# NoahVl/Explaining-In-Style-Reproducibility-Study

Hardware: AMD Instinct MI355X
Metric: StylEx G+D+enc train-step images/sec @256px (higher is better)
Workload: dtype bf16; 1 GPU; FFHQ-shaped 256x256 StylEx, batch 32/GPU, GAE=2 (noise+encoder micro-steps), GP every 4th step, ResNet-18 classifier; image_size=256, batch_per_gpu=32, start_step=0, gradient_accumulate_every=2, global_batch=32, parallelism=dp1

## Files before the change

### explaining-in-style-reproducibility-study_amd/csrc/fused_bwd.hip

```cpp
#include <hip/hip_runtime.h>
#include <stdint.h>
#include <stdlib.h>

#include "stylex_internal.h"

namespace {

constexpr int NT = 256;

template <int K>
struct Acc {
    float4 v[K];
    __device__ __forceinline__ void zero() {
#pragma unroll
        for (int k = 0; k < K; ++k) v[k] = make_float4(0.f, 0.f, 0.f, 0.f);
    }
};

template <int K>
__device__ __forceinline__ void block_reduce_store(Acc<K>& a, float* smem, int cv, int prow, int CV, int rpp, int C,
                                                   float* partial_row , bool active) {
    float4* s4 = reinterpret_cast<float4*>(smem);
    if (active) {
#pragma unroll
// ... 441 lines not shown
                        int nchunks, int act_dtype, void* stream) {
    if (act_dtype != 0 && act_dtype != 1) return STYLEX_EINVAL;
    if (!x || !t || !s || !partial || !ok_shape(sh, nchunks)) return STYLEX_EINVAL;
    int HW = (int)(sh[1] * sh[2]), C = (int)sh[3];
    if (glue_wide(act_dtype, C) && al16(x) && al16(t) && al16(s) && al16(gx) && al16(partial)) {
        hipLaunchKernelGGL(scale_reduce_wide_kernel, dim3(nchunks, (unsigned)sh[0]), dim3(NT8), reduce_smem8(C, 1),
                           (hipStream_t)stream, x, t, s, gx, partial, HW, C, nchunks);
        return (int)hipGetLastError();
    }
    hipLaunchKernelGGL(scale_reduce_kernel, dim3(nchunks, (unsigned)sh[0]), dim3(NT), reduce_smem(C, 1),
                       (hipStream_t)stream, x, t, s, gx, partial, HW, C, nchunks, act_dtype);
    return (int)hipGetLastError();
}

}
```

### explaining-in-style-reproducibility-study_amd/stylex/hip_backend.py

```python
import os as _os

if _os.environ.get("STYLEX_MIOPEN_ALLOW_BWD_GTC", "0") != "1":
    _os.environ.setdefault("MIOPEN_DEBUG_CONV_IMPLICIT_GEMM_ASM_BWD_GTC_XDLOPS_NHWC", "0")

import atexit
import ctypes
import os
import weakref

import torch

import operand_cache
from operand_cache import mark_updated, packs, stamp as _gen, vectors

_HERE = os.path.dirname(os.path.abspath(__file__))
LIB_PATH = os.path.join(os.path.dirname(_HERE), "libstylex_hip.so")

F32, BF16, BF16_ACT = 0, 1, 2
EPI_BIAS, EPI_LRELU, EPI_OSCALE, EPI_NOISE, EPI_RESIDUAL, EPI_RELU, EPI_GATE, EPI_NOISE_NAT = 1, 2, 4, 8, 16, 32, 64, 128
EPI_MASK_OUT, EPI_GATE_MASK = 256, 512

_c_f = ctypes.c_void_p
_i64p = ctypes.POINTER(ctypes.c_int64)

# ... 55 lines not shown
    "stylex_bias_act_fwd": (ctypes.c_int, [_c_f, _c_f, _c_f, ctypes.c_int64, _c_f, _c_f, _c_f, _i64p, ctypes.c_int,
                                           ctypes.c_void_p]),
    "stylex_bias_act_bwd": (ctypes.c_int, [_c_f, _c_f, _c_f, _i64p, ctypes.c_int, ctypes.c_void_p]),
    "stylex_rowwise_sumsq": (ctypes.c_int, [_c_f, _c_f, _i64p, ctypes.c_void_p]),
    "stylex_reduce_chunks": (ctypes.c_int, [_i64p]),
    "stylex_act_bwd_reduce": (ctypes.c_int, [_c_f, _c_f, _c_f, _c_f, _i64p, ctypes.c_int, ctypes.c_int, ctypes.c_float,
                                             ctypes.c_int, ctypes.c_void_p]),
    "stylex_modconv_bwd_prep": (ctypes.c_int, [_c_f, _c_f, _c_f, ctypes.c_int64, _c_f, _c_f, _c_f, _c_f, _i64p,
                                               ctypes.c_int, ctypes.c_int, ctypes.c_int, ctypes.c_void_p]),
    "stylex_modconv_bwd_prep_scaled": (ctypes.c_int, [_c_f, _c_f, _c_f, ctypes.c_int64, _c_f, _c_f, _c_f, _c_f, _c_f, _i64p,
                                                      ctypes.c_int, ctypes.c_int, ctypes.c_int, ctypes.c_void_p]),
    "stylex_modconv_bwd_prep_nat": (ctypes.c_int, [_c_f, _c_f, _c_f, ctypes.c_int64, _c_f, _c_f, _c_f, _c_f, _c_f, _i64p,
                                                   ctypes.c_int, ctypes.c_int, ctypes.c_int, ctypes.c_void_p]),
    "stylex_scale_reduce": (ctypes.c_int, [_c_f, _c_f, _c_f, _c_f, _c_f, _i64p, ctypes.c_int, ctypes.c_int,
                                           ctypes.c_void_p]),
    "stylex_pad_rgb8": (ctypes.c_int, [_c_f, _c_f, _i64p, _i64p, ctypes.c_int, ctypes.c_void_p]),
    "stylex_affine_act_nchw_fwd": (ctypes.c_int, [_c_f, _c_f, _c_f, _c_f, _c_f, ctypes.c_int64, ctypes.c_int64, ctypes.c_int64,
                                                  ctypes.c_int, ctypes.c_void_p]),
    "stylex_affine_act_nchw_bwd": (ctypes.c_int, [_c_f, _c_f, _c_f, _c_f, _c_f, ctypes.c_int64, ctypes.c_int64, ctypes.c_int64,
                                                  ctypes.c_int, ctypes.c_void_p]),
    "stylex_affine_relu_maxpool_fwd": (ctypes.c_int, [_c_f, _c_f, _c_f, _c_f, _c_f, ctypes.c_int64, ctypes.c_int64,
                                                      ctypes.c_int64, ctypes.c_int64, ctypes.c_void_p]),
    "stylex_affine_relu_maxpool_bwd": (ctypes.c_int, [_c_f, _c_f, _c_f, _c_f, ctypes.c_int64, ctypes.c_int64, ctypes.c_int64,
                                                      ctypes.c_int64, ctypes.c_void_p]),
    "stylex_lpips_tap_nhwc_fwd": (ctypes.c_int, [_c_f, _c_f, _c_f, _c_f, _c_f, _c_f, ctypes.c_int64, ctypes.c_int64, ctypes.c_int64,
                                                 ctypes.c_int64, ctypes.c_void_p]),
    "stylex_lpips_tap_nhwc_bwd": (ctypes.c_int, [_c_f, _c_f, _c_f, _c_f, _c_f, _c_f, _c_f, _c_f, ctypes.c_int64, ctypes.c_int64,
                                                 ctypes.c_int64, ctypes.c_void_p]),
    "stylex_nchw_f32_to_nhwc_bf16": (ctypes.c_int, [_c_f, _c_f, ctypes.c_int64, ctypes.c_int64, ctypes.c_int64, ctypes.c_int,
                                                    ctypes.c_void_p]),
# ... 86 lines not shown
                                          ctypes.c_int64, _c_f, _c_f, ctypes.c_int64, ctypes.c_void_p]),
    "stylex_style_edit_max_k": (ctypes.c_int64, []),
    "stylex_style_edit_levels": (ctypes.c_int, [_c_f] * 9 + [ctypes.c_int64] * 5 + [ctypes.c_float, ctypes.c_void_p]),
    "stylex_timing_report": (ctypes.c_int, [ctypes.c_int, _i64p, ctypes.POINTER(ctypes.c_double),
                                            ctypes.POINTER(ctypes.c_double), ctypes.POINTER(ctypes.c_double)]),
}

_lib = None
_inited_devices = set()


class StylexHipError(RuntimeError):
    pass


OPTIONAL_SYMBOLS = frozenset(["stylex_modconv_bwd_prep_nat"])
_MISSING_OPTIONAL = set()


def has_symbol(name):
    load_library()
    return name not in _MISSING_OPTIONAL


def load_library(path=None):
    global _lib
    if _lib is not None:
        return _lib
    path = path or os.environ.get("STYLEX_HIP_LIB", LIB_PATH)
    if not os.path.isfile(path):
        raise StylexHipError("libstylex_hip.so not found at %s — run `python __graft_entry__.py build` "
# ... 1448 lines not shown

def torgb_bwd(x, gy, s1, w, want_gx=True):
    lib = _ensure_device(x)
    assert is_cl(x) and is_cl(gy) and gy.shape[1] == 4 and x.dtype == gy.dtype == torch.bfloat16
    b, c, h, wd = x.shape
    shp = _shape(b, h, wd, c)
    nch = lib.stylex_torgb_chunks(shp)
    partial = _empty((b, nch, 3, c), dtype=torch.float32, device=x.device)
    gx = empty_cl(tuple(x.shape), x) if want_gx else None
    s1, w = _f32(s1), _f32(w)
    _check(lib.stylex_torgb_bwd(_ptr(x), _ptr(gy), _ptr(s1), _ptr(w), _ptr(gx), _ptr(partial), shp, _stream()),
           "stylex_torgb_bwd")
    return gx, (partial.sum(dim=1) if nch > 1 else partial[:, 0])


_STYLE_EDIT_MAX_K = None


def style_edit_max_k():
    global _STYLE_EDIT_MAX_K
    if _STYLE_EDIT_MAX_K is None:
        _STYLE_EDIT_MAX_K = int(load_library().stylex_style_edit_max_k())
    return _STYLE_EDIT_MAX_K


def _host_i32(values, what):
    v = [int(i) for i in values]
    if not v:
        raise ValueError("style_edit_levels: %s is empty" % what)
    return v
# ... 293 lines not shown
```

### explaining-in-style-reproducibility-study_amd/stylex/networks.py

```python
import atexit
import math
from math import log2

import os

import torch
import torch.nn.functional as F
from torch import nn

import ops


def exists(v):
    return v is not None


_SIDE = {}
atexit.register(_SIDE.clear)


def _side_stream(t, which=0):
    import os

    if not t.is_cuda or os.environ.get("STYLEX_STREAMS", "1") == "0":
# ... 188 lines not shown
        self.to_style = nn.Linear(latent_dim, input_channel)
        self.conv = Conv2DMod(input_channel, 4 if rgba else 3, 1, demod=False)
        self.upsample = nn.Sequential(Upsample2x(), Blur()) if upsample else None

    def forward(self, x, prev_rgb, istyle, style=None, padded=False):
        style = self.to_style(istyle) if style is None else style
        if padded and not self.conv.demod:
            fused = ops.rgb_block(x, prev_rgb, style, self.conv.weight, exists(self.upsample))
            if fused is not None:
                return fused
        if exists(prev_rgb) and prev_rgb.shape[1] == 4 and self.conv.weight.shape[0] == 3:
            prev_rgb = prev_rgb[:, :3]
        x = self.conv(x, style)
        if exists(prev_rgb):
            x = x + prev_rgb
        if exists(self.upsample):
            x = self.upsample(x)
        return x


class GeneratorBlock(nn.Module):
    def __init__(self, latent_dim, input_channels, filters, upsample=True, upsample_rgb=True, rgba=False):
        super().__init__()
        self.input_channels, self.filters = input_channels, filters
        self.num_style_coords = input_channels + filters
        self.upsample = Upsample2x() if upsample else None
        self.to_style1 = nn.Linear(latent_dim, input_channels)
        self.to_noise1 = nn.Linear(1, filters)
        self.conv1 = Conv2DMod(input_channels, filters, 3)
        self.to_style2 = nn.Linear(latent_dim, filters)
# ... 9 lines not shown
        self._rgb_style = None
        if styles is None:
            fused = ops.style_affines(istyle, self.to_style1, self.to_style2, self.to_rgb.to_style)
            if fused is not None:
                style1, style2, self._rgb_style, coords = fused
            else:
                style1, style2 = self.to_style1(istyle), self.to_style2(istyle)
        else:
            style1, style2 = styles
        x = ops.modconv_noise_act(x, style1, self.conv1.weight, inoise, self.to_noise1.weight[:, 0],
                                  self.to_noise1.bias, demod=self.conv1.demod, eps=self.conv1.eps)
        x = ops.modconv_noise_act(x, style2, self.conv2.weight, inoise, self.to_noise2.weight[:, 0],
                                  self.to_noise2.bias, demod=self.conv2.demod, eps=self.conv2.eps)
        return x, (coords if coords is not None else torch.cat([style1, style2], dim=-1))

    def forward(self, x, prev_rgb, istyle, inoise):
        x, coords = self.forward_main(x, istyle, inoise)
        rgb = self.to_rgb(x, prev_rgb, istyle, style=self.__dict__.pop("_rgb_style", None))
        return x, rgb, coords


class DiscriminatorBlock(nn.Module):
    def __init__(self, input_channels, filters, downsample=True):
        super().__init__()
        self.conv_res = HipConv2d(input_channels, filters, 1, stride=(2 if downsample else 1))
        self.net = nn.Sequential(HipConv2d(input_channels, filters, 3, padding=1, act=True), _FusedAct(),
                                 HipConv2d(filters, filters, 3, padding=1, act=True), _FusedAct())
        self.downsample = nn.Sequential(Blur(), HipConv2d(filters, filters, 3, padding=1, stride=2)) if downsample else None

    def forward(self, x):
        fused = getattr(ops.impl(), "dblock", None)
# ... 53 lines not shown

    def first_activation(self, styles):
        if self.no_const:
            return ops.initial_block(styles, self.to_initial_block.weight)
        return self.initial_block.expand(styles.shape[0], -1, -1, -1)

    def forward(self, styles, input_noise, get_style_coords=False, block_inputs=None):
        x = self.initial_conv(self.first_activation(styles))
        rgb, coords = None, []
        per_layer = styles.unbind(1)
        for li, block in enumerate(self.blocks):
            if exists(self.attns[li]):
                x = self.attns[li](x)
            if block_inputs is not None:
                block_inputs.append((x, rgb))
            x, sc = block.forward_main(x, per_layer[li], input_noise)
            coords.append(sc)
            rgb = block.to_rgb(x, rgb, per_layer[li], style=block.__dict__.pop("_rgb_style", None), padded=True)
        if rgb.shape[1] == 4 and self.blocks[0].to_rgb.conv.filters == 3:
            rgb = rgb[:, :3]
        rgb = rgb.float()
        if get_style_coords:
            return rgb, torch.cat(coords, dim=1)
        return rgb


class DiscriminatorE(nn.Module):
    def __init__(self, image_size, network_capacity=16, fq_layers=[], fq_dict_size=256, attn_layers=[],
                 transparent=False, encoder=False, encoder_dim=512, fmap_max=512, conditional=False):
        super().__init__()
# ... 31 lines not shown
```

### explaining-in-style-reproducibility-study_amd/stylex/ops.py

```python
import collections
import math

import os

import torch
from contextlib import nullcontext as _nullcontext
import torch.nn.functional as F

import hip_backend as hb

_PRECISION = hb.F32


_NAMES = {"fp32": hb.F32, "f32": hb.F32, "bf16": hb.BF16_ACT, "bf16_f32act": hb.BF16}


def set_precision(name):
    global _PRECISION
    _PRECISION = _NAMES[name]


def get_precision():
    return {hb.F32: "fp32", hb.BF16_ACT: "bf16", hb.BF16: "bf16_f32act"}[_PRECISION]

# ... 574 lines not shown


class _RGBTailFast(torch.autograd.Function):

    @staticmethod
    def forward(ctx, rgb, prev):
        return hb.rgb_up_blur_add_fwd(_cl(rgb), _cl(prev) if prev is not None else None)

    @staticmethod
    @torch.autograd.function.once_differentiable
    def backward(ctx, gy):
        g = hb.rgb_up_blur_add_bwd(_cl(gy))
        return g, (g if ctx.needs_input_grad[1] else None)


class _BlurS2D(torch.autograd.Function):

    @staticmethod
    def forward(ctx, x):
        return hb.blur3x3_s2d_fwd(_cl(x))

    @staticmethod
    def backward(ctx, gy2):
        return _BlurS2DBwd.apply(gy2)


class _BlurS2DBwd(torch.autograd.Function):
    @staticmethod
    def forward(ctx, gy2):
        return hb.blur3x3_s2d_bwd(_cl(gy2))
# ... 389 lines not shown
    @staticmethod
    def rgb_block(x, prev_rgb, style, weight, upsample):
        if not fast_enabled() or os.environ.get("STYLEX_RGB_TAIL", "1") == "0":
            return None
        x = _act(x)
        if tuple(weight.shape[2:]) != (1, 1) or weight.shape[0] != 3 or not hb.torgb_ok(x):
            return None
        if prev_rgb is not None and (prev_rgb.shape[1] != 4 or prev_rgb.dtype != x.dtype):
            return None
        rgb = _ToRGBFast.apply(x, style + 1, weight)
        if upsample:
            return _RGBTailFast.apply(rgb, prev_rgb)
        return rgb if prev_rgb is None else rgb + prev_rgb

    @staticmethod
    def residual_merge(x, res):
        return (x + res) * (1 / math.sqrt(2))

    @staticmethod
    def dblock(x, conv_res, conv1, conv2, down):
        if not fast_enabled() or os.environ.get("STYLEX_DBLOCK", "1") == "0":
            return None
        if conv1.weight.shape[0] % 4 != 0:
            return None
        return _DBlockFast.apply(x, conv_res.weight, conv_res.bias, conv1.weight, conv1.bias, conv2.weight, conv2.bias,
                                 down.weight if down is not None else None, down.bias if down is not None else None,
                                 down is not None)

    @staticmethod
    def style_edit_levels(coords, smin, smax, sindex, direction, base_class, level_k, seg_start, shift_size):
# ... 387 lines not shown
```

### include/stylex_hip.h

```cpp
#ifndef STYLEX_HIP_H
#define STYLEX_HIP_H

#include <stdint.h>

#ifdef __cplusplus
extern "C" {
#endif

#define STYLEX_F32 0
#define STYLEX_BF16 1
#define STYLEX_BF16_ACT 2

#define STYLEX_EINVAL (-1)
#define STYLEX_EWORKSPACE (-2)

#define STYLEX_CONV_NSHAPE 11

#define STYLEX_EPI_BIAS 1
#define STYLEX_EPI_LRELU 2
#define STYLEX_EPI_OSCALE 4
#define STYLEX_EPI_NOISE 8
#define STYLEX_EPI_RESIDUAL 16
#define STYLEX_EPI_RELU 32
#define STYLEX_EPI_NOISE_NAT 128
// ... 155 lines not shown
int stylex_act_bwd_reduce(const void* dy, const void* y, void* dx, float* partial, const int64_t* shape, int nchunks,
                          int lrelu, float scale, int act_dtype, void* stream);
int stylex_modconv_bwd_prep(const void* gy, const void* y, const float* noise, int64_t noise_stride,
                            const float* noise_w, const float* noise_b, void* gz, float* partial,
                            const int64_t* shape, int nchunks, int lrelu, int act_dtype, void* stream);
int stylex_modconv_bwd_prep_scaled(const void* gy, const void* y, const float* noise, int64_t noise_stride,
                                   const float* noise_w, const float* noise_b, const float* gz_scale, void* gz,
                                   float* partial, const int64_t* shape, int nchunks, int lrelu, int act_dtype,
                                   void* stream);
int stylex_modconv_bwd_prep_nat(const void* gy, const void* y, const float* noise, int64_t noise_stride,
                                const float* noise_w, const float* noise_b, const float* gz_scale, void* gz,
                                float* partial, const int64_t* shape, int nchunks, int lrelu, int act_dtype,
                                void* stream);
int stylex_scale_reduce(const void* x, const void* t, const float* s, void* gx, float* partial, const int64_t* shape,
                        int nchunks, int act_dtype, void* stream);

int stylex_torgb_chunks(const int64_t* shape);
int stylex_torgb_fwd(const void* x, const float* s1, const float* w, void* y, const int64_t* shape, void* stream);
int stylex_torgb_bwd(const void* x, const void* gy, const float* s1, const float* w, void* gx, float* partial,
                     const int64_t* shape, void* stream);

int stylex_timing_enable(int on);
int stylex_timing_pause(int on);
int stylex_timing_report(int kernel_class, int64_t* launches, double* total_ms, double* total_flops,
                         double* total_bytes);
int stylex_timing_layers(int64_t* meta, double* vals, int64_t cap);
int stylex_timing_kernels(char* names, int64_t* meta, double* vals, int64_t cap);

#define STYLEX_ADAM_COPY_PACK 0
#define STYLEX_ADAM_COPY_PACK_S2D 1
// ... 85 lines not shown
```

Before: 1007 images/sec.

## Fuse generator block backward seams into top, mid and bottom kernels

Adds a custom autograd function for a whole generator block. Its backward pass uses three new fused HIP kernels. The top kernel combines the toRGB input gradient, the residual gradient add, the lrelu/noise prep and the demod sums. The mid kernel fuses the style-scale reduction with the next prep step. The bottom kernel merges the input scaling with the transposed bilinear 2x upsample, so the full-resolution gradient is never materialized. This removes several intermediate activation round-trips and kernel launches per block, at the cost of a lot of new code and different rounding points.

```diff
diff --git a/explaining-in-style-reproducibility-study_amd/csrc/fused_bwd.hip b/explaining-in-style-reproducibility-study_amd/csrc/fused_bwd.hip
--- a/explaining-in-style-reproducibility-study_amd/csrc/fused_bwd.hip
+++ b/explaining-in-style-reproducibility-study_amd/csrc/fused_bwd.hip
@@ -479,3 +479,477 @@
 }
 
 }
+
+namespace {
+
+template <int V>
+struct LN {
+    float e[V];
+};
+template <int V>
+__device__ __forceinline__ LN<V> ldv(const void* p, long off, int bf) {
+    LN<V> r;
+    if constexpr (V == 8) {
+        const L8 t = ld8(p, off);
+#pragma unroll
+        for (int e = 0; e < 8; ++e) r.e[e] = t.e[e];
+    } else {
+        const float4 t = act_ld4(p, off, bf);
+        r.e[0] = t.x; r.e[1] = t.y; r.e[2] = t.z; r.e[3] = t.w;
+    }
+    return r;
+}
+template <int V>
+__device__ __forceinline__ void stv(void* p, long off, const LN<V>& v, int bf) {
+    if constexpr (V == 8) {
+        *reinterpret_cast<uint4*>(reinterpret_cast<unsigned short*>(p) + off) =
+            make_uint4(act_pack2(v.e[0], v.e[1]), act_pack2(v.e[2], v.e[3]), act_pack2(v.e[4], v.e[5]), act_pack2(v.e[6], v.e[7]));
+    } else {
+        act_st4(p, off, make_float4(v.e[0], v.e[1], v.e[2], v.e[3]), bf);
+    }
+}
+template <int V>
+__device__ __forceinline__ LN<V> ldpv(const float* p) {
+    LN<V> r;
+#pragma unroll
+    for (int q = 0; q < V / 4; ++q) {
+        const float4 t = ldp4(p + 4 * q);
+        r.e[4 * q] = t.x; r.e[4 * q + 1] = t.y; r.e[4 * q + 2] = t.z; r.e[4 * q + 3] = t.w;
+    }
+    return r;
+}
+template <int V>
+__device__ __forceinline__ void rndv(LN<V>& v, int bf) {
+    if (V == 8 || bf) {
+#pragma unroll
+        for (int e = 0; e < V; e += 2) {
+            const unsigned u = act_pack2(v.e[e], v.e[e + 1]);
+            v.e[e] = act_lo(u);
+            v.e[e + 1] = act_hi(u);
+        }
+    }
+}
+
+template <int V>
+__device__ __forceinline__ Geo8 make_geov(int n, int C, int nchunks) {
+    Geo8 g;
+    g.CV = C / V;
+    g.rpp = NT / (C >> 2);
+    g.cv = threadIdx.x % g.CV;
+    g.prow = threadIdx.x / g.CV;
+    g.active = g.prow < g.rpp;
+    g.b = blockIdx.y;
+    const long per = ((long)n + nchunks - 1) / nchunks;
+    const long pb = (long)blockIdx.x * per;
+    g.p_begin = (int)(pb < n ? pb : n);
+    g.p_end = (int)(pb + per < n ? pb + per : n);
+    return g;
+}
+
+template <int V, int K, int K0>
+__device__ __forceinline__ void block_reduce_storev(const LN<V> (&a)[K], float* smem, const Geo8& g, int C, float* row0,
+                                                    float* row1) {
+    constexpr int Q = V / 4;
+    float4* s4 = reinterpret_cast<float4*>(smem);
+    if (g.active) {
+#pragma unroll
+        for (int k = 0; k < K; ++k) {
+            const int at = ((k * g.rpp + g.prow) * g.CV + g.cv) * Q;
+#pragma unroll
+            for (int q = 0; q < Q; ++q) s4[at + q] = make_float4(a[k].e[4 * q], a[k].e[4 * q + 1], a[k].e[4 * q + 2], a[k].e[4 * q + 3]);
+        }
+    }
+    __syncthreads();
+    if (g.active && g.prow == 0) {
+#pragma unroll
+        for (int k = 0; k < K; ++k) {
+            float4 t[Q];
+#pragma unroll
+            for (int q = 0; q < Q; ++q) t[q] = make_float4(0.f, 0.f, 0.f, 0.f);
+            for (int r = 0; r < g.rpp; ++r) {
+                const int at = ((k * g.rpp + r) * g.CV + g.cv) * Q;
+#pragma unroll
+                for (int q = 0; q < Q; ++q) {
+                    const float4 x = s4[at + q];
+                    t[q].x += x.x; t[q].y += x.y; t[q].z += x.z; t[q].w += x.w;
+                }
+            }
+            float4* d = reinterpret_cast<float4*>((k < K0 ? row0 + (long)k * C : row1 + (long)(k - K0) * C) + g.cv * V);
+#pragma unroll
+            for (int q = 0; q < Q; ++q) d[q] = t[q];
+        }
+    }
+}
+
+template <int V>
+__device__ __forceinline__ void prep_pixel(LN<V>& q, const LN<V>& y, float nz, const LN<V>& w8, const LN<V>& b8, const LN<V>& d8,
+                                           bool scaled, int lrelu, void* gz, long o, int bf, LN<V>& a0, LN<V>& a1, LN<V>& a2,
+                                           bool live) {
+    LN<V> t = y, s;
+#pragma unroll
+    for (int e = 0; e < V; ++e) {
+        if (lrelu) {
+            const float g = q.e[e];
+            q.e[e] = y.e[e] > 0.f ? g : 0.2f * g;
+            t.e[e] = y.e[e] > 0.f ? y.e[e] : 5.f * y.e[e];
+        }
+        s.e[e] = scaled ? q.e[e] * d8.e[e] : q.e[e];
+    }
+    if (live) {
+        stv<V>(gz, o, s, bf);
+#pragma unroll
+        for (int e = 0; e < V; ++e) {
+            a0.e[e] += q.e[e] * (t.e[e] - (nz * w8.e[e] + b8.e[e]));
+            a1.e[e] += q.e[e] * nz;
+            a2.e[e] += q.e[e];
+        }
+    }
+}
+
+template <int V>
+__global__ __launch_bounds__(V == 8 ? NT8 : NT) void gblock_bwd_mid_kernel(
+    const void* __restrict__ t, const void* __restrict__ y, const float* __restrict__ s, const float* __restrict__ noise, int ns,
+    const float* __restrict__ nw, const float* __restrict__ nb, void* __restrict__ gz, float* __restrict__ partial,
+    float* __restrict__ partial_gs, int H, int W, int C, int nchunks, int lrelu, const float* __restrict__ gz_scale, int bf) {
+    extern __shared__ __attribute__((aligned(16))) float smem[];
+    const int HW = H * W;
+    const Geo8 g = make_geov<V>(HW, C, nchunks);
+    LN<V> a[4] = {};
+    if (g.active) {
+        const int c = g.cv * V;
+        LN<V> w8 = {}, b8 = {}, d8 = {};
+        if (noise) {
+            w8 = ldpv<V>(nw + c);
+            b8 = ldpv<V>(nb + c);
+        }
+        if (gz_scale) d8 = ldpv<V>(gz_scale + (long)g.b * C + c);
+        const LN<V> s8 = ldpv<V>(s + (long)g.b * C + c);
+        const long step = (long)g.rpp * C;
+        long o = ((long)g.b * HW + g.p_begin + g.prow) * C + c;
+        PixWalk pw(g.p_begin + g.prow, g.rpp, W);
+        for (int p = g.p_begin + g.prow; p < g.p_end; p += 2 * g.rpp, o += 2 * step, pw.advance()) {
+            const bool two = p + g.rpp < g.p_end;
+            const long o1 = two ? o + step : o;
+            const int h0 = pw.h, w0 = pw.w;
+            pw.advance();
+            const int h1 = two ? pw.h : h0, w1 = two ? pw.w : w0;
+            LN<V> t0 = ldv<V>(t, o, bf), t1 = ldv<V>(t, o1, bf);
+            const LN<V> y0 = ldv<V>(y, o, bf), y1 = ldv<V>(y, o1, bf);
+            float nz0 = 0.f, nz1 = 0.f;
+            if (noise) {
+                nz0 = noise[noise_off(g.b, ns, h0, w0, 1)];
+                nz1 = noise[noise_off(g.b, ns, h1, w1, 1)];
+            }
+#pragma unroll
+            for (int e = 0; e < V; ++e) a[3].e[e] += y0.e[e] * t0.e[e];
+            if (two) {
+#pragma unroll
+                for (int e = 0; e < V; ++e) a[3].e[e] += y1.e[e] * t1.e[e];
+            }
+#pragma unroll
+            for (int e = 0; e < V; ++e) {
+                t0.e[e] *= s8.e[e];
+                t1.e[e] *= s8.e[e];
+            }
+            rndv<V>(t0, bf);
+            rndv<V>(t1, bf);
+            prep_pixel<V>(t0, y0, nz0, w8, b8, d8, gz_scale != nullptr, lrelu, gz, o, bf, a[0], a[1], a[2], true);
+            prep_pixel<V>(t1, y1, nz1, w8, b8, d8, gz_scale != nullptr, lrelu, gz, o1, bf, a[0], a[1], a[2], two);
+        }
+    }
+    const long blk = (long)g.b * nchunks + blockIdx.x;
+    block_reduce_storev<V, 4, 3>(a, smem, g, C, partial + blk * 3 * C, partial_gs + blk * C);
+}
+
+template <bool WANT_T>
+__global__ __launch_bounds__(NT8) void gblock_bwd_top_kernel(
+    const void* __restrict__ gx_in, const uint2* __restrict__ grgb, const void* __restrict__ y, const float* __restrict__ s_rgb,
+    const float* __restrict__ w_rgb, const float* __restrict__ noise, int ns, const float* __restrict__ nw,
+    const float* __restrict__ nb, void* __restrict__ gz, float* __restrict__ partial, float* __restrict__ partial_t, int H, int W,
+    int C, int nchunks, int lrelu, const float* __restrict__ gz_scale) {
+    extern __shared__ __attribute__((aligned(16))) float smem[];
+    const int HW = H * W;
+    const Geo8 g = make_geov<8>(HW, C, nchunks);
+    constexpr int K = WANT_T ? 6 : 3;
+    LN<8> a[K] = {};
+    if (g.active) {
+        const int c = g.cv * 8;
+        LN<8> w8 = {}, b8 = {}, d8 = {};
+        if (noise) {
+            w8 = ldpv<8>(nw + c);
+            b8 = ldpv<8>(nb + c);
+        }
+        if (gz_scale) d8 = ldpv<8>(gz_scale + (long)g.b * C + c);
+        LN<8> m[3];
+        {
+            const LN<8> sr = ldpv<8>(s_rgb + (long)g.b * C + c);
+#pragma unroll
+            for (int n = 0; n < 3; ++n) {
+                m[n] = ldpv<8>(w_rgb + (long)n * C + c);
+#pragma unroll
+                for (int e = 0; e < 8; ++e) m[n].e[e] *= sr.e[e];
+            }
+        }
+        const uint2* gr = grgb + (long)g.b * HW;
+        const long step = (long)g.rpp * C;
+        long o = ((long)g.b * HW + g.p_begin + g.prow) * C + c;
+        PixWalk pw(g.p_begin + g.prow, g.rpp, W);
+        for (int p = g.p_begin + g.prow; p < g.p_end; p += 2 * g.rpp, o += 2 * step, pw.advance()) {
+            const bool two = p + g.rpp < g.p_end;
+            const long o1 = two ? o + step : o;
+            const int p1 = two ? p + g.rpp : p;
+            const int h0 = pw.h, w0 = pw.w;
+            pw.advance();
+            const int h1 = two ? pw.h : h0, w1 = two ? pw.w : w0;
+            const uint2 r0 = gr[p], r1 = gr[p1];
+            const LN<8> y0 = ldv<8>(y, o, 1), y1 = ldv<8>(y, o1, 1);
+            LN<8> x0 = {}, x1 = {};
+            if (gx_in) {
+                x0 = ldv<8>(gx_in, o, 1);
+                x1 = ldv<8>(gx_in, o1, 1);
+            }
+            float nz0 = 0.f, nz1 = 0.f;
+            if (noise) {
+                nz0 = noise[noise_off(g.b, ns, h0, w0, 1)];
+                nz1 = noise[noise_off(g.b, ns, h1, w1, 1)];
+            }
+            const float g00 = act_lo(r0.x), g01 = act_hi(r0.x), g02 = act_lo(r0.y);
+            const float g10 = act_lo(r1.x), g11 = act_hi(r1.x), g12 = act_lo(r1.y);
+            LN<8> q0, q1;
+#pragma unroll
+            for (int e = 0; e < 8; ++e) {
+                q0.e[e] = fmaf(g02, m[2].e[e], fmaf(g00, m[0].e[e], g01 * m[1].e[e]));
+                q1.e[e] = fmaf(g12, m[2].e[e], fmaf(g10, m[0].e[e], g11 * m[1].e[e]));
+            }
+            rndv<8>(q0, 1);
+            rndv<8>(q1, 1);
+            if (gx_in) {
+#pragma unroll
+                for (int e = 0; e < 8; ++e) {
+                    q0.e[e] += x0.e[e];
+                    q1.e[e] += x1.e[e];
+                }
+                rndv<8>(q0, 1);
+                rndv<8>(q1, 1);
+            }
+            if constexpr (WANT_T) {
+#pragma unroll
+                for (int e = 0; e < 8; ++e) {
+                    a[K - 3].e[e] = fmaf(y0.e[e], g00, a[K - 3].e[e]);
+                    a[K - 2].e[e] = fmaf(y0.e[e], g01, a[K - 2].e[e]);
+                    a[K - 1].e[e] = fmaf(y0.e[e], g02, a[K - 1].e[e]);
+                }
+                if (two) {
+#pragma unroll
+                    for (int e = 0; e < 8; ++e) {
+                        a[K - 3].e[e] = fmaf(y1.e[e], g10, a[K - 3].e[e]);
+                        a[K - 2].e[e] = fmaf(y1.e[e], g11, a[K - 2].e[e]);
+                        a[K - 1].e[e] = fmaf(y1.e[e], g12, a[K - 1].e[e]);
+                    }
+                }
+            }
+            prep_pixel<8>(q0, y0, nz0, w8, b8, d8, gz_scale != nullptr, lrelu, gz, o, 1, a[0], a[1], a[2], true);
+            prep_pixel<8>(q1, y1, nz1, w8, b8, d8, gz_scale != nullptr, lrelu, gz, o1, 1, a[0], a[1], a[2], two);
+        }
+    }
+    const long blk = (long)g.b * nchunks + blockIdx.x;
+    block_reduce_storev<8, K, 3>(a, smem, g, C, partial + blk * 3 * C, WANT_T ? partial_t + blk * 3 * C : nullptr);
+}
+
+__device__ __forceinline__ float up2_coef(int o, int i, int n) {
+    const int k = o >> 1;
+    int lo, hi;
+    float wh;
+    if (o & 1) {
+        lo = k;
+        hi = min(k + 1, n - 1);
+        wh = 0.25f;
+    } else {
+        lo = max(k - 1, 0);
+        hi = k;
+        wh = 0.75f;
+    }
+    return (lo == i ? 1.f - wh : 0.f) + (hi == i ? wh : 0.f);
+}
+
+template <int V, int ROWS, bool SUM>
+__global__ __launch_bounds__(V == 8 ? NT8 : NT) void gblock_bwd_bottom_kernel(
+    const void* __restrict__ t, const void* __restrict__ xup, const float* __restrict__ s, void* __restrict__ gxl,
+    float* __restrict__ partial, int H, int W, int C, int nchunks) {
+    extern __shared__ __attribute__((aligned(16))) float smem[];
+    constexpr int bf = V == 8;
+    const int strips = (H + ROWS - 1) / ROWS;
+    const Geo8 g = make_geov<V>(strips * W, C, nchunks);
+    LN<V> a[1] = {};
+    if (g.active) {
+        const int c = g.cv * V;
+        const LN<V> s8 = ldpv<V>(s + (long)g.b * C + c);
+        const long rs = (long)W * C, ors = 2 * rs;
+        const long hi_base = (long)g.b * 2 * H * ors + c;
+        for (int q = g.p_begin + g.prow; q < g.p_end; q += g.rpp) {
+            const int hs = q / W, iw = q - hs * W, h0 = hs * ROWS;
+            const int own_end = min(2 * (h0 + ROWS), 2 * H);
+            long oc[4];
+            float cw[4];
+#pragma unroll
+            for (int e = 0; e < 4; ++e) {
+                const int ow = 2 * iw + e - 1;
+                const bool in = ow >= 0 && ow < 2 * W;
+                cw[e] = in ? up2_coef(ow, iw, W) : 0.f;
+                oc[e] = (long)min(max(ow, 0), 2 * W - 1) * C;
+            }
+            auto ldrow = [&](int oh, uint4 (&v)[4]) {
+                const bool own = oh >= 2 * h0 && oh < own_end;
+                const long ro = hi_base + (long)min(max(oh, 0), 2 * H - 1) * ors;
+#pragma unroll
+                for (int e = 0; e < 4; ++e) {
+                    LN<V> tv = ldv<V>(t, ro + oc[e], bf);
+                    if (SUM && (e == 1 || e == 2) && own) {
+                        const LN<V> xv = ldv<V>(xup, ro + oc[e], bf);
+#pragma unroll
+                        for (int k = 0; k < V; ++k) a[0].e[k] += xv.e[k] * tv.e[k];
+                    }
+#pragma unroll
+                    for (int k = 0; k < V; ++k) tv.e[k] *= s8.e[k];
+                    if constexpr (V == 8)
+                        v[e] = make_uint4(act_pack2(tv.e[0], tv.e[1]), act_pack2(tv.e[2], tv.e[3]), act_pack2(tv.e[4], tv.e[5]),
+                                          act_pack2(tv.e[6], tv.e[7]));
+                    else
+                        v[e] = make_uint4(__float_as_uint(tv.e[0]), __float_as_uint(tv.e[1]), __float_as_uint(tv.e[2]),
+                                          __float_as_uint(tv.e[3]));
+                }
+            };
+            uint4 win[4][4];
+            ldrow(2 * h0 - 1, win[0]);
+            ldrow(2 * h0, win[1]);
+#pragma unroll
+            for (int r = 0; r < ROWS; ++r) {
+                const int ih = h0 + r;
+                if (ih >= H) break;
+                ldrow(2 * ih + 1, win[2]);
+                ldrow(2 * ih + 2, win[3]);
+                LN<V> acc = {};
+#pragma unroll
+                for (int k = 0; k < 4; ++k) {
+                    const int oh = 2 * ih + k - 1;
+                    const float ch = (oh >= 0 && oh < 2 * H) ? up2_coef(oh, ih, H) : 0.f;
+                    if (ch == 0.f) continue;
+#pragma unroll
+                    for (int e = 0; e < 4; ++e) {
+                        if (cw[e] == 0.f) continue;
+                        const uint4 u = win[k][e];
+                        const float wgt = ch * cw[e];
+                        if constexpr (V == 8) {
+                            acc.e[0] = fmaf(wgt, act_lo(u.x), acc.e[0]); acc.e[1] = fmaf(wgt, act_hi(u.x), acc.e[1]);
+                            acc.e[2] = fmaf(wgt, act_lo(u.y), acc.e[2]); acc.e[3] = fmaf(wgt, act_hi(u.y), acc.e[3]);
+                            acc.e[4] = fmaf(wgt, act_lo(u.z), acc.e[4]); acc.e[5] = fmaf(wgt, act_hi(u.z), acc.e[5]);
+                            acc.e[6] = fmaf(wgt, act_lo(u.w), acc.e[6]); acc.e[7] = fmaf(wgt, act_hi(u.w), acc.e[7]);
+                        } else {
+                            acc.e[0] = fmaf(wgt, __uint_as_float(u.x), acc.e[0]); acc.e[1] = fmaf(wgt, __uint_as_float(u.y), acc.e[1]);
+                            acc.e[2] = fmaf(wgt, __uint_as_float(u.z), acc.e[2]); acc.e[3] = fmaf(wgt, __uint_as_float(u.w), acc.e[3]);
+                        }
+                    }
+                }
+                stv<V>(gxl, ((long)g.b * H + ih) * rs + (long)iw * C + c, acc, bf);
+#pragma unroll
+                for (int e = 0; e < 4; ++e) {
+                    win[0][e] = win[2][e];
+                    win[1][e] = win[3][e];
+                }
+            }
+        }
+    }
+    if constexpr (SUM) block_reduce_storev<V, 1, 1>(a, smem, g, C, partial + ((long)g.b * nchunks + blockIdx.x) * C, nullptr);
+}
+
+constexpr int GB_ROWS = 8;
+inline size_t reduce_smemv(int K) { return (size_t)K * NT * 16; }
+
+inline bool ok_noise(const float* noise, int64_t stride, const float* nw, const float* nb, const int64_t* sh) {
+    return !noise || (nw && nb && stride >= sh[1] && stride >= sh[2]);
+}
+
+}
+
+extern "C" {
+
+int stylex_gblock_bwd_top(const void* g_x, const void* g_rgb, const void* y, const float* s_rgb, const float* w_rgb,
+                          const float* noise, int64_t noise_stride, const float* noise_w, const float* noise_b,
+                          const float* gz_scale, void* gz, float* partial, float* partial_t, const int64_t* sh,
+                          int nchunks, int lrelu, int act_dtype, void* stream) {
+    if (act_dtype != 0 && act_dtype != 1) return STYLEX_EINVAL;
+    if (lrelu != 0 && lrelu != 1) return STYLEX_EINVAL;
+    if (!g_rgb || !y || !s_rgb || !w_rgb || !gz || !partial || !ok_shape(sh, nchunks)) return STYLEX_EINVAL;
+    if (!ok_noise(noise, noise_stride, noise_w, noise_b, sh)) return STYLEX_EINVAL;
+    const int C = (int)sh[3];
+    if (act_dtype != 1 || C % 8 != 0) return STYLEX_NOT_APPLICABLE;
+    if (!(al16(g_x) && al16(y) && al16(gz) && al16(partial) && al16(partial_t) && al16(noise_w) && al16(noise_b) &&
+          al16(gz_scale) && al16(s_rgb) && al16(w_rgb)) || (reinterpret_cast<uintptr_t>(g_rgb) & 7))
+        return STYLEX_EINVAL;
+    if (partial_t)
+        hipLaunchKernelGGL(gblock_bwd_top_kernel<true>, dim3(nchunks, (unsigned)sh[0]), dim3(NT8), reduce_smemv(6),
+                           (hipStream_t)stream, g_x, (const uint2*)g_rgb, y, s_rgb, w_rgb, noise, (int)noise_stride, noise_w,
+                           noise_b, gz, partial, partial_t, (int)sh[1], (int)sh[2], C, nchunks, lrelu, gz_scale);
+    else
+        hipLaunchKernelGGL(gblock_bwd_top_kernel<false>, dim3(nchunks, (unsigned)sh[0]), dim3(NT8), reduce_smemv(3),
+                           (hipStream_t)stream, g_x, (const uint2*)g_rgb, y, s_rgb, w_rgb, noise, (int)noise_stride, noise_w,
+                           noise_b, gz, partial, partial_t, (int)sh[1], (int)sh[2], C, nchunks, lrelu, gz_scale);
+    return (int)hipGetLastError();
+}
+
+int stylex_gblock_bwd_mid(const void* t, const void* y, const float* s, const float* noise, int64_t noise_stride,
+                          const float* noise_w, const float* noise_b, const float* gz_scale, void* gz, float* partial,
+                          float* partial_gs, const int64_t* sh, int nchunks, int lrelu, int act_dtype, void* stream) {
+    if (act_dtype != 0 && act_dtype != 1) return STYLEX_EINVAL;
+    if (lrelu != 0 && lrelu != 1) return STYLEX_EINVAL;
+    if (!t || !y || !s || !gz || !partial || !partial_gs || !ok_shape(sh, nchunks)) return STYLEX_EINVAL;
+    if (!ok_noise(noise, noise_stride, noise_w, noise_b, sh)) return STYLEX_EINVAL;
+    if (!(al16(s) && al16(partial) && al16(partial_gs) && al16(noise_w) && al16(noise_b) && al16(gz_scale))) return STYLEX_EINVAL;
+    const int C = (int)sh[3];
+    if (glue_wide(act_dtype, C) && al16(t) && al16(y) && al16(gz)) {
+        hipLaunchKernelGGL(gblock_bwd_mid_kernel<8>, dim3(nchunks, (unsigned)sh[0]), dim3(NT8), reduce_smemv(4),
+                           (hipStream_t)stream, t, y, s, noise, (int)noise_stride, noise_w, noise_b, gz, partial, partial_gs,
+                           (int)sh[1], (int)sh[2], C, nchunks, lrelu, gz_scale, 1);
+        return (int)hipGetLastError();
+    }
+    hipLaunchKernelGGL(gblock_bwd_mid_kernel<4>, dim3(nchunks, (unsigned)sh[0]), dim3(NT), reduce_smemv(4), (hipStream_t)stream,
+                       t, y, s, noise, (int)noise_stride, noise_w, noise_b, gz, partial, partial_gs, (int)sh[1], (int)sh[2], C,
+                       nchunks, lrelu, gz_scale, act_dtype);
+    return (int)hipGetLastError();
+}
+
+int stylex_gblock_bwd_bottom_chunks(const int64_t* sh) {
+    if (sh[1] <= 0 || sh[2] <= 0 || sh[3] < 4 || sh[3] > 1024) return 1;
+    const long items = ((sh[1] + GB_ROWS - 1) / GB_ROWS) * sh[2];
+    const long rpp = NT / (sh[3] >> 2);
+    const long n = (items + rpp - 1) / rpp;
+    return (int)(n > 65535 ? 65535 : n);
+}
+
+int stylex_gblock_bwd_bottom(const void* t, const void* x_up, const float* s, void* gx_low, float* partial,
+                             const int64_t* sh, int nchunks, int act_dtype, void* stream) {
+    if (act_dtype != 0 && act_dtype != 1) return STYLEX_EINVAL;
+    if (!t || !s || !gx_low || !ok_shape(sh, nchunks) || (x_up == nullptr) != (partial == nullptr)) return STYLEX_EINVAL;
+    if (sh[1] * sh[2] >= (1L << 26)) return STYLEX_EINVAL;
+    if (!(al16(t) && al16(x_up) && al16(s) && al16(gx_low) && al16(partial))) return STYLEX_EINVAL;
+    const int H = (int)sh[1], W = (int)sh[2], C = (int)sh[3];
+    if (act_dtype == 1) {
+        if (C % 8 != 0) return STYLEX_NOT_APPLICABLE;
+        if (partial)
+            hipLaunchKernelGGL((gblock_bwd_bottom_kernel<8, GB_ROWS, true>), dim3(nchunks, (unsigned)sh[0]), dim3(NT8),
+                               reduce_smemv(1), (hipStream_t)stream, t, x_up, s, gx_low, partial, H, W, C, nchunks);
+        else
+            hipLaunchKernelGGL((gblock_bwd_bottom_kernel<8, GB_ROWS, false>), dim3(nchunks, (unsigned)sh[0]), dim3(NT8), 0,
+                               (hipStream_t)stream, t, x_up, s, gx_low, partial, H, W, C, nchunks);
+    } else {
+        if (partial)
+            hipLaunchKernelGGL((gblock_bwd_bottom_kernel<4, GB_ROWS, true>), dim3(nchunks, (unsigned)sh[0]), dim3(NT),
+                               reduce_smemv(1), (hipStream_t)stream, t, x_up, s, gx_low, partial, H, W, C, nchunks);
+        else
+            hipLaunchKernelGGL((gblock_bwd_bottom_kernel<4, GB_ROWS, false>), dim3(nchunks, (unsigned)sh[0]), dim3(NT), 0,
+                               (hipStream_t)stream, t, x_up, s, gx_low, partial, H, W, C, nchunks);
+    }
+    return (int)hipGetLastError();
+}
+
+}
diff --git a/explaining-in-style-reproducibility-study_amd/stylex/hip_backend.py b/explaining-in-style-reproducibility-study_amd/stylex/hip_backend.py
--- a/explaining-in-style-reproducibility-study_amd/stylex/hip_backend.py
+++ b/explaining-in-style-reproducibility-study_amd/stylex/hip_backend.py
@@ -93,6 +93,13 @@
                                                    ctypes.c_int, ctypes.c_int, ctypes.c_int, ctypes.c_void_p]),
     "stylex_scale_reduce": (ctypes.c_int, [_c_f, _c_f, _c_f, _c_f, _c_f, _i64p, ctypes.c_int, ctypes.c_int,
                                            ctypes.c_void_p]),
+    "stylex_gblock_bwd_top": (ctypes.c_int, [_c_f, _c_f, _c_f, _c_f, _c_f, _c_f, ctypes.c_int64, _c_f, _c_f, _c_f, _c_f, _c_f,
+                                             _c_f, _i64p, ctypes.c_int, ctypes.c_int, ctypes.c_int, ctypes.c_void_p]),
+    "stylex_gblock_bwd_mid": (ctypes.c_int, [_c_f, _c_f, _c_f, _c_f, ctypes.c_int64, _c_f, _c_f, _c_f, _c_f, _c_f, _c_f, _i64p,
+                                             ctypes.c_int, ctypes.c_int, ctypes.c_int, ctypes.c_void_p]),
+    "stylex_gblock_bwd_bottom_chunks": (ctypes.c_int, [_i64p]),
+    "stylex_gblock_bwd_bottom": (ctypes.c_int, [_c_f, _c_f, _c_f, _c_f, _c_f, _i64p, ctypes.c_int, ctypes.c_int,
+                                                ctypes.c_void_p]),
     "stylex_pad_rgb8": (ctypes.c_int, [_c_f, _c_f, _i64p, _i64p, ctypes.c_int, ctypes.c_void_p]),
     "stylex_affine_act_nchw_fwd": (ctypes.c_int, [_c_f, _c_f, _c_f, _c_f, _c_f, ctypes.c_int64, ctypes.c_int64, ctypes.c_int64,
                                                   ctypes.c_int, ctypes.c_void_p]),
@@ -209,7 +216,8 @@
     pass
 
 
-OPTIONAL_SYMBOLS = frozenset(["stylex_modconv_bwd_prep_nat"])
+OPTIONAL_SYMBOLS = frozenset(["stylex_modconv_bwd_prep_nat", "stylex_gblock_bwd_top", "stylex_gblock_bwd_mid",
+                              "stylex_gblock_bwd_bottom_chunks", "stylex_gblock_bwd_bottom"])
 _MISSING_OPTIONAL = set()
 
 
@@ -1688,6 +1696,68 @@
     return gx, (partial.sum(dim=1) if nch > 1 else partial[:, 0])
 
 
+GBLOCK_SYMBOLS = ("stylex_gblock_bwd_top", "stylex_gblock_bwd_mid", "stylex_gblock_bwd_bottom_chunks", "stylex_gblock_bwd_bottom")
+
+
+def gblock_seams_available():
+    return all(has_symbol(n) for n in GBLOCK_SYMBOLS)
+
+
+def _prep_args(noise, noise_w, noise_b, gz_scale):
+    noise, noise_w, noise_b, gz_scale = _f32(noise), _f32(noise_w), _f32(noise_b), _f32(gz_scale)
+    return noise, noise_w, noise_b, gz_scale, (noise.shape[1] if noise is not None else 0)
+
+
+def gblock_bwd_top(g_x, g_rgb, y, s_rgb, w_rgb, noise_nat, noise_w, noise_b, lrelu, gz_scale=None, want_t=True):
+    lib = _ensure_device(y)
+    assert is_cl(y) and is_cl(g_rgb) and g_rgb.shape[1] == 4 and y.dtype == g_rgb.dtype == torch.bfloat16
+    assert g_x is None or (is_cl(g_x) and g_x.dtype == y.dtype and g_x.shape == y.shape)
+    b, c, h, w = y.shape
+    shp = _shape(b, h, w, c)
+    nch = lib.stylex_reduce_chunks(shp)
+    partial = _empty((b, nch, 3, c), dtype=torch.float32, device=y.device)
+    partial_t = _empty((b, nch, 3, c), dtype=torch.float32, device=y.device) if want_t else None
+    gz = empty_cl(tuple(y.shape), y)
+    noise, noise_w, noise_b, gz_scale, ns = _prep_args(noise_nat, noise_w, noise_b, gz_scale)
+    s_rgb, w_rgb = _f32(s_rgb), _f32(w_rgb)
+    _check(lib.stylex_gblock_bwd_top(_ptr(g_x), _ptr(g_rgb), _ptr(y), _ptr(s_rgb), _ptr(w_rgb), _ptr(noise), ns, _ptr(noise_w),
+                                     _ptr(noise_b), _ptr(gz_scale), _ptr(gz), _ptr(partial), _ptr(partial_t), shp, nch,
+                                     int(bool(lrelu)), _adt(y), _stream()), "stylex_gblock_bwd_top")
+    return gz, partial.sum(dim=1), (None if not want_t else partial_t.sum(dim=1) if nch > 1 else partial_t[:, 0])
+
+
+def gblock_bwd_mid(t, y, s, noise_nat, noise_w, noise_b, lrelu, gz_scale=None):
+    lib = _ensure_device(y)
+    assert is_cl(y) and is_cl(t) and y.dtype == t.dtype and y.shape == t.shape
+    b, c, h, w = y.shape
+    shp = _shape(b, h, w, c)
+    nch = lib.stylex_reduce_chunks(shp)
+    partial = _empty((b, nch, 3, c), dtype=torch.float32, device=y.device)
+    partial_gs = _empty((b, nch, c), dtype=torch.float32, device=y.device)
+    gz = empty_cl(tuple(y.shape), y)
+    noise, noise_w, noise_b, gz_scale, ns = _prep_args(noise_nat, noise_w, noise_b, gz_scale)
+    s = _f32(s)
+    _check(lib.stylex_gblock_bwd_mid(_ptr(t), _ptr(y), _ptr(s), _ptr(noise), ns, _ptr(noise_w), _ptr(noise_b), _ptr(gz_scale),
+                                     _ptr(gz), _ptr(partial), _ptr(partial_gs), shp, nch, int(bool(lrelu)), _adt(y), _stream()),
+           "stylex_gblock_bwd_mid")
+    return gz, partial.sum(dim=1), partial_gs.sum(dim=1)
+
+
+def gblock_bwd_bottom(t, x_up, s):
+    lib = _ensure_device(t)
+    assert is_cl(t) and (x_up is None or (is_cl(x_up) and t.dtype == x_up.dtype and t.shape == x_up.shape))
+    b, c, h2, w2 = t.shape
+    assert h2 % 2 == 0 and w2 % 2 == 0
+    shp = _shape(b, h2 // 2, w2 // 2, c)
+    nch = lib.stylex_gblock_bwd_bottom_chunks(shp)
+    partial = _empty((b, nch, c), dtype=torch.float32, device=t.device) if x_up is not None else None
+    gx = empty_cl((b, c, h2 // 2, w2 // 2), t)
+    s = _f32(s)
+    _check(lib.stylex_gblock_bwd_bottom(_ptr(t), _ptr(x_up), _ptr(s), _ptr(gx), _ptr(partial), shp, nch, _adt(t), _stream()),
+           "stylex_gblock_bwd_bottom")
+    return gx, (partial.sum(dim=1) if partial is not None else None)
+
+
 _STYLE_EDIT_MAX_K = None
 
 
diff --git a/explaining-in-style-reproducibility-study_amd/stylex/networks.py b/explaining-in-style-reproducibility-study_amd/stylex/networks.py
--- a/explaining-in-style-reproducibility-study_amd/stylex/networks.py
+++ b/explaining-in-style-reproducibility-study_amd/stylex/networks.py
@@ -226,6 +226,16 @@
         x = self.conv(x, style)
         if exists(prev_rgb):
             x = x + prev_rgb
+        if exists(self.upsample):
+            x = self.upsample(x)
+        return x
+
+    def finish(self, rgb4, prev_rgb, padded=False):
+        if padded:
+            return ops.impl().rgb_tail(rgb4, prev_rgb, exists(self.upsample))
+        x = rgb4[:, :3]
+        if exists(prev_rgb):
+            x = x + (prev_rgb[:, :3] if prev_rgb.shape[1] == 4 else prev_rgb)
         if exists(self.upsample):
             x = self.upsample(x)
         return x
@@ -265,7 +275,25 @@
                                   self.to_noise2.bias, demod=self.conv2.demod, eps=self.conv2.eps)
         return x, (coords if coords is not None else torch.cat([style1, style2], dim=-1))
 
+    def forward_fused(self, x, prev_rgb, istyle, inoise, padded=False):
+        rgb_conv = self.to_rgb.conv
+        if not exists(self.upsample) or getattr(ops.impl(), "gblock", None) is None:
+            return None
+        if not ops.gblock_ok(x, self.input_channels, self.filters, rgb_conv.weight,
+                             (self.conv1.demod, self.conv2.demod, not rgb_conv.demod), inoise):
+            return None
+        if padded and exists(prev_rgb) and (prev_rgb.shape[1] != 4 or prev_rgb.dtype != x.dtype):
+            return None
+        fused = ops.style_affines(istyle, self.to_style1, self.to_style2, self.to_rgb.to_style)
+        if fused is None:
+            return None
+        x, rgb = ops.impl().gblock(x, fused[:3], inoise, self.conv1, self.conv2, self.to_noise1, self.to_noise2, rgb_conv)
+        return x, self.to_rgb.finish(rgb, prev_rgb, padded), fused[3]
+
     def forward(self, x, prev_rgb, istyle, inoise):
+        fused = self.forward_fused(x, prev_rgb, istyle, inoise)
+        if fused is not None:
+            return fused
         x, coords = self.forward_main(x, istyle, inoise)
         rgb = self.to_rgb(x, prev_rgb, istyle, style=self.__dict__.pop("_rgb_style", None))
         return x, rgb, coords
@@ -349,6 +377,12 @@
                 x = self.attns[li](x)
             if block_inputs is not None:
                 block_inputs.append((x, rgb))
+            fused = None if (self.no_const or exists(self.attns[li])) else block.forward_fused(
+                x, rgb, per_layer[li], input_noise, padded=True)
+            if fused is not None:
+                x, rgb, sc = fused
+                coords.append(sc)
+                continue
             x, sc = block.forward_main(x, per_layer[li], input_noise)
             coords.append(sc)
             rgb = block.to_rgb(x, rgb, per_layer[li], style=block.__dict__.pop("_rgb_style", None), padded=True)
diff --git a/explaining-in-style-reproducibility-study_amd/stylex/ops.py b/explaining-in-style-reproducibility-study_amd/stylex/ops.py
--- a/explaining-in-style-reproducibility-study_amd/stylex/ops.py
+++ b/explaining-in-style-reproducibility-study_amd/stylex/ops.py
@@ -612,6 +612,119 @@
         return g, (g if ctx.needs_input_grad[1] else None)
 
 
+GBLOCK_SEAMS = ("top", "mid", "bottom")
+_GBLOCK_DEFAULT_SEAMS = frozenset(GBLOCK_SEAMS)
+
+
+def _gblock_seams():
+    v = os.environ.get("STYLEX_GBLOCK_SEAMS")
+    if v is None:
+        return _GBLOCK_DEFAULT_SEAMS
+    seams = frozenset(s for s in v.replace(" ", "").split(",") if s)
+    if not seams <= frozenset(GBLOCK_SEAMS):
+        raise ValueError("STYLEX_GBLOCK_SEAMS=%r: a subset of %s" % (v, ",".join(GBLOCK_SEAMS)))
+    return seams
+
+
+def gblock_ok(x, cin, filters, rgb_weight, demod, inoise):
+    if _IMPL is not HipOps or not fast_enabled() or os.environ.get("STYLEX_GBLOCK", "1") == "0":
+        return False
+    if _PRECISION != hb.BF16_ACT or not x.is_cuda or x.dtype != torch.bfloat16 or x.dim() != 4 or x.shape[1] != cin:
+        return False
+    if cin % 8 or filters % 8 or cin > 1024 or not (8 <= filters <= 512 and filters & (filters - 1) == 0):
+        return False
+    if not all(demod) or tuple(rgb_weight.shape) != (3, filters, 1, 1):
+        return False
+    if 4 * x.shape[2] * x.shape[3] <= 64 or inoise.shape[1] % 4 or inoise.shape[1] != inoise.shape[2]:
+        return False
+    if os.environ.get("STYLEX_NOISE_NAT", "1") == "0" or os.environ.get("STYLEX_TORGB", "1") == "0":
+        return False
+    if os.environ.get("STYLEX_RGB_TAIL", "1") == "0" or os.environ.get("STYLEX_GLUE_WIDE", "1") == "0":
+        return False
+    return hb.gblock_seams_available()
+
+
+class _GBlockFast(torch.autograd.Function):
+
+    @staticmethod
+    def forward(ctx, x, s11, d1, w1, nw1, nb1, s12, d2, w2, nw2, nb2, s_rgb, w_rgb, nat):
+        pad = (w1.shape[2] - 1) // 2
+        x_up = hb.upsample2x_fwd(_cl(x))
+        y1 = hb.conv2d_fwd(x_up, w1, 1, pad, _PRECISION, in_scale=s11, out_scale=d1, noise=nat, noise_w=nw1, noise_b=nb1,
+                           lrelu=True, noise_natural=True)
+        y2 = hb.conv2d_fwd(y1, w2, 1, pad, _PRECISION, in_scale=s12, out_scale=d2, noise=nat, noise_w=nw2, noise_b=nb2,
+                           lrelu=True, noise_natural=True)
+        rgb = hb.torgb_fwd(y2, s_rgb, w_rgb)
+        ctx.save_for_backward(x_up, y1, y2, s11, d1, w1, nw1, nb1, s12, d2, w2, nw2, nb2, s_rgb, w_rgb, nat)
+        ctx.pad, ctx.seams = pad, _gblock_seams()
+        ctx.fold = os.environ.get("STYLEX_FOLD_D", "1") != "0"
+        ctx.fused_sums = os.environ.get("STYLEX_GBLOCK_SUMS", "") == "fused"
+        ctx.set_materialize_grads(False)
+        return y2, rgb
+
+    @staticmethod
+    @torch.autograd.function.once_differentiable
+    def backward(ctx, g_x, g_rgb):
+        x_up, y1, y2, s11, d1, w1, nw1, nb1, s12, d2, w2, nw2, nb2, s_rgb, w_rgb, nat = ctx.saved_tensors
+        pad, seams, fold, need, fused_sums = ctx.pad, ctx.seams, ctx.fold, ctx.needs_input_grad, ctx.fused_sums
+        g_x = _cl(g_x) if g_x is not None else None
+        prep = lambda gy, y, nw, nb, d: hb.modconv_bwd_prep(gy, y, nat, nw, nb, True, gz_scale=d if fold else None,
+                                                            noise_natural=True)
+
+        def conv_grads(gz, x_in, s, d, w, want_w):
+            t = hb.conv2d_bwd_data(gz, w, tuple(x_in.shape), 1, pad, _PRECISION, in_scale=None if fold else d)
+            gw = hb.conv2d_bwd_weight(x_in, gz, tuple(w.shape), 1, pad, _PRECISION, x_scale=s,
+                                      dy_scale=None if fold else d) if want_w else None
+            return t, gw
+
+        gs_rgb = gw_rgb = None
+        if g_rgb is None:
+            if g_x is None:
+                return (None,) * 14
+            gz2, sums2 = prep(g_x, y2, nw2, nb2, d2)
+        else:
+            g_rgb = _cl(g_rgb)
+            if "top" in seams:
+                gz2, sums2, t_rgb = hb.gblock_bwd_top(g_x, g_rgb, y2, s_rgb, w_rgb, nat, nw2, nb2, True,
+                                                      gz_scale=d2 if fold else None, want_t=fused_sums)
+                if t_rgb is None and (need[11] or need[12]):
+                    _, t_rgb = hb.torgb_bwd(y2, g_rgb, s_rgb, w_rgb, want_gx=False)
+            else:
+                gy2, t_rgb = hb.torgb_bwd(y2, g_rgb, s_rgb, w_rgb, want_gx=True)
+                if g_x is not None:
+                    gy2 = gy2 + g_x
+                gz2, sums2 = prep(gy2, y2, nw2, nb2, d2)
+                del gy2
+            if need[11]:
+                gs_rgb = (t_rgb * w_rgb.reshape(1, 3, -1).float()).sum(dim=1)
+            if need[12]:
+                gw_rgb = (t_rgb * s_rgb.float()[:, None, :]).sum(dim=0).reshape(w_rgb.shape).to(w_rgb.dtype)
+        del g_x, g_rgb
+        gd2 = sums2[:, 0] / d2
+        gnw2, gnb2 = sums2[:, 1:3].sum(0)
+        t2, gw2 = conv_grads(gz2, y1, s12, d2, w2, need[8])
+        del gz2
+        if "mid" in seams:
+            gz1, sums1, gs12 = hb.gblock_bwd_mid(t2, y1, s12, nat, nw1, nb1, True, gz_scale=d1 if fold else None)
+        else:
+            gx1, gs12 = hb.scale_reduce(y1, t2, s12, want_gx=True)
+            gz1, sums1 = prep(gx1, y1, nw1, nb1, d1)
+            del gx1
+        del t2
+        gd1 = sums1[:, 0] / d1
+        gnw1, gnb1 = sums1[:, 1:3].sum(0)
+        t1, gw1 = conv_grads(gz1, x_up, s11, d1, w1, need[3])
+        del gz1
+        if "bottom" in seams:
+            gx, gs11 = hb.gblock_bwd_bottom(t1, x_up if fused_sums else None, s11)
+            if gs11 is None:
+                _, gs11 = hb.scale_reduce(x_up, t1, s11, want_gx=False)
+        else:
+            gx_up, gs11 = hb.scale_reduce(x_up, t1, s11, want_gx=True)
+            gx = hb.upsample2x_bwd(gx_up)
+        return (gx if need[0] else None, gs11, gd1, gw1, gnw1, gnb1, gs12, gd2, gw2, gnw2, gnb2, gs_rgb, gw_rgb, None)
+
+
 class _BlurS2D(torch.autograd.Function):
 
     @staticmethod
@@ -1031,6 +1144,20 @@
         return rgb if prev_rgb is None else rgb + prev_rgb
 
     @staticmethod
+    def rgb_tail(rgb, prev_rgb, upsample):
+        if upsample:
+            return _RGBTailFast.apply(rgb, prev_rgb)
+        return rgb if prev_rgb is None else rgb + prev_rgb
+
+    @staticmethod
+    def gblock(x, styles, inoise, conv1, conv2, to_noise1, to_noise2, rgb_conv):
+        s11, d1 = mod_coeffs(styles[0], conv1.weight, True, conv1.eps)
+        s12, d2 = mod_coeffs(styles[1], conv2.weight, True, conv2.eps)
+        return _GBlockFast.apply(x, s11, d1, conv1.weight, to_noise1.weight[:, 0], to_noise1.bias, s12, d2, conv2.weight,
+                                 to_noise2.weight[:, 0], to_noise2.bias, styles[2] + 1, rgb_conv.weight,
+                                 _natural_noise(inoise))
+
+    @staticmethod
     def residual_merge(x, res):
         return (x + res) * (1 / math.sqrt(2))
 
diff --git a/include/stylex_hip.h b/include/stylex_hip.h
--- a/include/stylex_hip.h
+++ b/include/stylex_hip.h
@@ -193,6 +193,17 @@
                                 void* stream);
 int stylex_scale_reduce(const void* x, const void* t, const float* s, void* gx, float* partial, const int64_t* shape,
                         int nchunks, int act_dtype, void* stream);
+
+int stylex_gblock_bwd_top(const void* g_x, const void* g_rgb, const void* y, const float* s_rgb, const float* w_rgb,
+                          const float* noise, int64_t noise_stride, const float* noise_w, const float* noise_b,
+                          const float* gz_scale, void* gz, float* partial, float* partial_t, const int64_t* shape,
+                          int nchunks, int lrelu, int act_dtype, void* stream);
+int stylex_gblock_bwd_mid(const void* t, const void* y, const float* s, const float* noise, int64_t noise_stride,
+                          const float* noise_w, const float* noise_b, const float* gz_scale, void* gz, float* partial,
+                          float* partial_gs, const int64_t* shape, int nchunks, int lrelu, int act_dtype, void* stream);
+int stylex_gblock_bwd_bottom_chunks(const int64_t* shape);
+int stylex_gblock_bwd_bottom(const void* t, const void* x_up, const float* s, void* gx_low, float* partial,
+                             const int64_t* shape, int nchunks, int act_dtype, void* stream);
 
 int stylex_torgb_chunks(const int64_t* shape);
 int stylex_torgb_fwd(const void* x, const float* s1, const float* w, void* y, const int64_t* shape, void* stream);
```

Result: no change. 1017 images/sec (median of 6 runs) (+1.0%).
